# mmeidlinger/lut_ldpc

Measured on AMD Instinct MI355X. Metric: decoded codewords/sec, DVB-S2 N=64800 4-bit LUT 50-iter, higher is better.
Workload: dtype u8

## Files before the change

lut_ldpc_amd/csrc/hip/kernels_common.hpp:

```cpp
#pragma once
#ifndef __HIPCC_RTC__
#include <hip/hip_runtime.h>
#include <stdint.h>
#else
typedef unsigned char uint8_t;
typedef unsigned short uint16_t;
typedef unsigned int uint32_t;
typedef unsigned long long uint64_t;
typedef short int16_t;
typedef int int32_t;
typedef long long int64_t;
#endif

namespace lutldpc {

constexpr int kRowBytes = 256;
constexpr int kTileFrames = kRowBytes;
constexpr int kWave = 64;
constexpr int kMaxSeg = 32;

constexpr uint32_t ST_ACTIVE = 0, ST_DONE_PSC = 1, ST_DONE_PISC = 2, ST_PAD = 3;
constexpr uint32_t ST_DONE_SAVED = 4;

struct PassSeg {
    int32_t block_begin;
    int32_t n_nodes;
    int32_t node_off;
    int32_t deg;
    int32_t op_off;
    int32_t n_ops;
    int32_t tab_off;
    int32_t tab_bytes;
    int32_t n_in, n_out, n_slots;
    int32_t fast;
};

struct PassParams {
    int32_t n_seg;
    int32_t blocks_per_group;
    int32_t nodes_per_block;
    int32_t G;
    int32_t E;
    int32_t N;
    int32_t nz;
    int32_t check;
    int32_t write_hard;
    int32_t slots_lds;
    int32_t vfail_stride_w;
    PassSeg seg[kMaxSeg];
};

template <int PACK>
__device__ __forceinline__ uint32_t unpack_half(uint32_t x, int h) {
    if constexpr (PACK == 1) return x;
    else return h ? ((x >> 4) & 0x0F0F0F0Fu) : (x & 0x0F0F0F0Fu);
}
template <int PACK>
__device__ __forceinline__ uint32_t pack_halves(const uint32_t (&r)[PACK]) {
    if constexpr (PACK == 1) return r[0];
    else return r[0] | (r[1] << 4);
}
template <int PACK>
__device__ __forceinline__ uint32_t pack_masks(const uint32_t (&m)[PACK]) {
    if constexpr (PACK == 1) return m[0];
    else return (m[0] & 0x0F0F0F0Fu) | (m[1] & 0xF0F0F0F0u);
}
template <int PACK>
__device__ __forceinline__ int frame_word(int g, int lane, int h) { return (g * kWave + lane) * PACK + h; }

__device__ __forceinline__ uint32_t swar_lt(uint32_t x, uint32_t t) {
    uint32_t d = (x | 0x80808080u) - t * 0x01010101u;
    return (~d >> 7) & 0x01010101u;
}
__device__ __forceinline__ uint32_t swar_zero_mask(uint32_t x) {
    uint32_t nz = ((x & 0x7F7F7F7Fu) + 0x7F7F7F7Fu) | x;
    uint32_t z = (~nz >> 7) & 0x01010101u;
    return z * 0xFFu;
}
__device__ __forceinline__ uint32_t bfi(uint32_t m, uint32_t a, uint32_t b) { return __builtin_amdgcn_bitop3_b32(m, a, b, (0xCC & 0xF0) | (0xAA & 0x0F)); }

using rsrc_t = __amdgpu_buffer_rsrc_t;
__device__ __forceinline__ rsrc_t make_rsrc(const void *p, uint32_t bytes) {
    return __builtin_amdgcn_make_buffer_rsrc(const_cast<void *>(p), 0, (int)bytes, 0x00020000);
}
#ifndef LUTLDPC_LD_AUX
#define LUTLDPC_LD_AUX 2
#endif
#ifndef LUTLDPC_ST_AUX
#define LUTLDPC_ST_AUX 2
#endif
__device__ __forceinline__ uint32_t ld_row(rsrc_t r, uint32_t row_off, uint32_t lane4) {
    return (uint32_t)__builtin_amdgcn_raw_buffer_load_b32(r, (int)lane4, (int)row_off, LUTLDPC_LD_AUX);
}
__device__ __forceinline__ void st_row(rsrc_t r, uint32_t row_off, uint32_t lane4, uint32_t v) {
    __builtin_amdgcn_raw_buffer_store_b32(v, r, (int)lane4, (int)row_off, LUTLDPC_ST_AUX);
}

__device__ __forceinline__ void pipeline_entry_fence() {
    asm volatile("" ::: "memory");
    __builtin_amdgcn_sched_barrier(0);
    __builtin_amdgcn_s_waitcnt(0x0F70);
    __builtin_amdgcn_sched_barrier(0);
    asm volatile("" ::: "memory");
}

__device__ __forceinline__ bool wave_all_zero(uint32_t x) { return __ballot(x != 0) == 0ull; }

template <int PACK>
__device__ __forceinline__ bool load_active(const uint32_t *__restrict__ state_w, int g, int lane, uint32_t (&amask)[PACK]) {
    uint32_t any = 0;
#pragma unroll
    for (int h = 0; h < PACK; h++) { amask[h] = swar_zero_mask(state_w[frame_word<PACK>(g, lane, h)]); any |= amask[h]; }
    return wave_all_zero(any);
}

template <int PACK>
__device__ __forceinline__ void store_blend(uint32_t *p, uint32_t val, uint32_t old, uint32_t smask) {
    *p = bfi(smask, val, old);
}
template <int PACK>
__device__ __forceinline__ void store_row_masked(uint32_t *p, uint32_t val, uint32_t smask) {
    if (smask == 0xFFFFFFFFu) *p = val;
    else if (smask) *p = bfi(smask, val, *p);
}

constexpr int kVfailSlots = 32;
template <int PACK>
__device__ __forceinline__ void flag_frames(uint32_t *__restrict__ vfail_w, int stride_w, int g, int lane, const uint32_t (&fail)[PACK], const uint32_t (&amask)[PACK]) {
    uint32_t *slot = vfail_w + (size_t)(blockIdx.x & (kVfailSlots - 1)) * (size_t)stride_w;
#pragma unroll
    for (int h = 0; h < PACK; h++) {
        const uint32_t f = fail[h] & amask[h] & 0x01010101u;
        if (f) atomicOr(&slot[frame_word<PACK>(g, lane, h)], f);
    }
}

constexpr int kFastMaxTables = 32;
constexpr int kFastTableStride = 256;

struct FastParams {
    int32_t n_nodes, node_off, nodes_per_wave, waves_per_group;
    int32_t idx_off;
    int32_t G, E, N;
    int32_t g0;
    int32_t nz;
    int32_t shift_msg;
    int32_t check, write_hard;
    int32_t deg;
    int32_t n_tables;
    int32_t tab_off[kFastMaxTables];
    int32_t tab_len[kFastMaxTables];
    int32_t tab_shift[kFastMaxTables];
    int32_t nib;
    int32_t vfail_stride_w;
    int32_t vfail_off_w;
};
struct ChainParams {
    int32_t on;
    int32_t idx_off;
    int32_t tab_off, tab_len, tab_shift;
    int32_t check, hard, vfail_off_w, sbit_out;
};

__device__ __forceinline__ uint32_t lshl_or(uint32_t x, int s, uint32_t y) {
    uint32_t r;
    asm("v_lshl_or_b32 %0, %1, %2, %3" : "=v"(r) : "v"(x), "s"(s), "v"(y));
    return r;
}

__device__ __forceinline__ uint32_t xad(uint32_t a, uint32_t b, uint32_t c) {
    uint32_t r;
    asm("v_xad_u32 %0, %1, %2, %3" : "=v"(r) : "v"(a), "s"(b), "v"(c));
    return r;
}
__device__ __forceinline__ uint32_t xor3(uint32_t a, uint32_t b, uint32_t c) { return __builtin_amdgcn_bitop3_b32(a, b, c, 0xF0 ^ 0xCC ^ 0xAA); }
__device__ __forceinline__ uint32_t xor_or(uint32_t a, uint32_t b, uint32_t c) { return __builtin_amdgcn_bitop3_b32(a, b, c, (0xF0 ^ 0xCC) | 0xAA); }

#ifndef __HIPCC_RTC__
constexpr size_t kMaxKernelArgBytes = 128;
template <typename... KArgs, typename... Args>
inline void launch_k(void (*kernel)(KArgs...), dim3 grid, dim3 block, size_t shmem, hipStream_t stream, Args &&...args) {
    static_assert((((sizeof(KArgs) + 7) / 8 * 8) + ... + 0) <= kMaxKernelArgBytes, "kernel argument segment above 128 bytes: pass the structure through device memory");
    hipLaunchKernelGGL(kernel, grid, block, shmem, stream, static_cast<KArgs>(args)...);
}
#endif

__device__ __forceinline__ int find_seg(const PassParams &P, int b) {
    int s = 0;
#pragma unroll 1
    for (int i = 1; i < P.n_seg; i++) if (b >= P.seg[i].block_begin) s = i;
    return s;
}

}
```

lut_ldpc_amd/csrc/hip/kernels_fast.hpp:

```cpp
#pragma once
#include "kernels_common.hpp"
#include "lut_program.hpp"

#include <utility>

namespace lutldpc {

constexpr int kCnAllButOneMaxDeg = 16;
template <int DEG, int UNR, int PACK, bool CHAIN, typename PT, bool FIRST = false, int ABO = kCnAllButOneMaxDeg>
__device__ __forceinline__ void cn_minsum_body(
    const PT &P, int block, uint8_t *msgs, const uint32_t *__restrict__ state_w, uint32_t *__restrict__ vfail_w,
    const int32_t *__restrict__ fast_idx, const ChainParams CH = ChainParams{}, uint8_t *lds_tab = nullptr,
    const uint8_t *cha = nullptr, const uint8_t *__restrict__ tables = nullptr, uint8_t *hard = nullptr, const uint8_t *msg0 = nullptr)
{
    static_assert(!CHAIN || (UNR == 1 && DEG >= 2), "chain fusion: one check per step");
    if constexpr (CHAIN) {
        const int i = threadIdx.x;
        if (CH.on && i < CH.tab_len / 4) reinterpret_cast<uint32_t *>(lds_tab)[i] = reinterpret_cast<const uint32_t *>(tables + CH.tab_off)[i];
        __syncthreads();
    }
    const int lane = threadIdx.x & 63;
    const int wave = __builtin_amdgcn_readfirstlane(block * 4 + (threadIdx.x >> 6));
    const int gl = wave / P.waves_per_group;
    if (gl >= P.G) return;
    const int chunk = wave - gl * P.waves_per_group;
    const int g = gl + P.g0;
    uint32_t amask[PACK];
    if (load_active<PACK>(state_w, g, lane, amask)) return;
    const uint32_t smask = pack_masks<PACK>(amask);
    const bool all_active = __ballot(smask != 0xFFFFFFFFu) == 0ull;
    const rsrc_t base = make_rsrc(msgs + (size_t)g * (size_t)P.E * kRowBytes, (uint32_t)P.E * kRowBytes);
    const uint32_t lane4 = (uint32_t)lane * 4u;
    const int32_t *edges = fast_idx + P.idx_off;
    const int32_t *nodes = edges;
    rsrc_t nbase = base;
    if constexpr (FIRST) {
        nodes = fast_idx + P.nidx_off;
        nbase = make_rsrc(msg0 + (size_t)g * (size_t)P.N * kRowBytes, (uint32_t)P.N * kRowBytes);
    }
    const int first = chunk * P.nodes_per_wave;
    int last = first + P.nodes_per_wave;
    if (last > P.n_nodes) last = P.n_nodes;
    constexpr uint32_t ONE = PACK == 2 ? 0x11111111u : 0x01010101u;
    const int sbit = __builtin_ctz((unsigned)P.nz);
    const uint32_t SB = (uint32_t)P.nz * ONE, LOW = SB - ONE;
    const uint32_t odd = (DEG & 1) ? SB : 0u;
    uint32_t failw = 0;

    const int32_t *links = CHAIN ? fast_idx + CH.idx_off : nullptr;
    const rsrc_t cbase = CHAIN ? make_rsrc(cha + (size_t)g * (size_t)P.N * kRowBytes, (uint32_t)P.N * kRowBytes) : base;
    int lb = 0, lf = 0, lbn = 0, lfn = 0;
    uint32_t xc = 0, xcn = 0;
    uint32_t pend = 0, pend_old = 0, chainfail = 0;
    int pend_e = 0;
    auto fetch = [&](int i, uint32_t (&xx)[UNR][DEG], int (&ee)[UNR][DEG]) {
#pragma unroll
        for (int u = 0; u < UNR; u++) {
            const int ii = (i + u < last) ? i + u : last - 1;
#pragma unroll
            for (int k = 0; k < DEG; k++) ee[u][k] = edges[(size_t)ii * DEG + k];
            if constexpr (CHAIN) { lbn = links[2 * (size_t)ii]; lfn = links[2 * (size_t)ii + 1]; }
        }
#pragma unroll
        for (int u = 0; u < UNR; u++) {
            const uint32_t off = lane4 | ((i + u < last) ? 0u : 0x80000000u);
#pragma unroll
            for (int k = 0; k < DEG; k++) {
                if constexpr (FIRST) {
                    const int ii = (i + u < last) ? i + u : last - 1;
                    xx[u][k] = ld_row(nbase, (uint32_t)nodes[(size_t)ii * DEG + k] * kRowBytes, off);
                } else xx[u][k] = ld_row(base, (uint32_t)ee[u][k] * kRowBytes, off);
            }
            if constexpr (CHAIN) xcn = ld_row(cbase, (uint32_t)(lbn > 0 ? lbn - 1 : 0) * kRowBytes, (i + u < last && lbn > 0 && CH.on) ? lane4 : (lane4 | 0x80000000u));
        }
    };
    auto to_mc = [&](uint32_t xh) -> uint32_t {
        const uint32_t pos = xh & SB;
        return (xh ^ (pos - (pos >> sbit))) & LOW;
    };
    auto from_mc = [&](uint32_t mc, uint32_t po) -> uint32_t {
        return xor_or(mc, po - (po >> sbit), po);
    };
    auto eval = [&](int i, const uint32_t (&x)[UNR][DEG], const int (&e)[UNR][DEG]) {
#pragma unroll
        for (int u = 0; u < UNR; u++) {
            if (i + u >= last) break;
            uint32_t r[DEG];
            uint32_t tn;
            if constexpr (DEG <= ABO) {
            auto mx = [&](uint32_t a, uint32_t b) -> uint32_t {
                const uint32_t gt = xad(b, LOW, a) & SB;
                return bfi(gt - (gt >> sbit), a, b);
            };
            uint32_t mcs[DEG], spp = 0;
#pragma unroll
            for (int k = 0; k < DEG; k++) {
                const uint32_t xh = x[u][k];
                mcs[k] = to_mc(xh);
                if (k & 1) spp = xor3(spp, x[u][k - 1], xh);
                else if (k == DEG - 1) spp ^= xh;
            }
            tn = (spp ^ odd) & SB;
            uint32_t oc[DEG];
            if constexpr (DEG == 1) oc[0] = 0u;
            else if constexpr (DEG == 2) { oc[0] = mcs[1]; oc[1] = mcs[0]; }
            else {
                uint32_t suf[DEG];
                suf[DEG - 1] = mcs[DEG - 1];
#pragma unroll
                for (int k = DEG - 2; k >= 1; k--) suf[k] = mx(mcs[k], suf[k + 1]);
                uint32_t pre = mcs[0];
                oc[0] = suf[1];
#pragma unroll
                for (int k = 1; k <= DEG - 2; k++) { oc[k] = mx(pre, suf[k + 1]); pre = mx(pre, mcs[k]); }
                oc[DEG - 1] = pre;
            }
#pragma unroll
            for (int k = 0; k < DEG; k++) r[k] = from_mc(oc[k], (tn ^ x[u][k]) & SB);
            } else {
            uint32_t min1 = LOW, min2 = LOW, spp = 0;
            uint32_t mg[DEG];
#pragma unroll
            for (int k = 0; k < DEG; k++) {
                const uint32_t xh = x[u][k];
                const uint32_t mag = to_mc(xh) ^ LOW;
                spp ^= xh;
                mg[k] = mag;
                if (k == 0) {
                    min1 = mag;
                } else {
                    const uint32_t g1 = ((mag | SB) - min1) & SB;
                    const uint32_t k1 = g1 - (g1 >> sbit);
                    const uint32_t lo = bfi(k1, min1, mag);
                    const uint32_t hi = mag ^ min1 ^ lo;
                    if (k == 1) {
                        min2 = hi;
                    } else {
                        const uint32_t g2 = ((min2 | SB) - hi) & SB;
                        const uint32_t k2 = g2 - (g2 >> sbit);
                        min2 = bfi(k2, hi, min2);
                    }
                    min1 = lo;
                }
            }
            tn = (spp ^ odd) & SB;
            const uint32_t m1c = min1 ^ LOW, m2c = min2 ^ LOW;
#pragma unroll
            for (int k = 0; k < DEG; k++) {
                const uint32_t eq = ~(((mg[k] ^ min1) | SB) - ONE) & SB;
                const uint32_t ke = eq - (eq >> sbit);
                r[k] = from_mc(bfi(ke, m2c, m1c), (tn ^ x[u][k]) & SB);
            }
            }
            if (P.check) failw |= tn >> sbit;
            if constexpr (CHAIN) {
                [[maybe_unused]] constexpr int F = 4 * PACK, BITS = 8 / PACK;
                if (lb && CH.hard) {
                    const uint32_t neg = (~x[u][0] >> sbit) & ONE;
                    store_row_masked<PACK>(reinterpret_cast<uint32_t *>(hard + ((size_t)g * (size_t)P.N + (size_t)(lb - 1)) * kRowBytes + lane4), neg, smask);
                }
                if (lb && CH.on) {
                    uint32_t o_prev = 0, o_this = 0, dif = 0;
                    if constexpr (PACK == 2) {
                        constexpr uint32_t NIB = 0x0F0F0F0Fu;
                        const uint32_t c_lo = xc & NIB, c_hi = (xc >> 4) & NIB;
                        const uint32_t ia_lo = lshl_or(c_lo, CH.tab_shift, pend & NIB), ia_hi = lshl_or(c_hi, CH.tab_shift, (pend >> 4) & NIB);
                        const uint32_t ib_lo = lshl_or(c_lo, CH.tab_shift, r[0] & NIB), ib_hi = lshl_or(c_hi, CH.tab_shift, (r[0] >> 4) & NIB);
#pragma unroll 1
                        for (int s = 0; s < 32; s += 8) {
                            const uint32_t vp0 = lds_tab[__builtin_amdgcn_ubfe(ib_lo, (uint32_t)s, 8u)], vt0 = lds_tab[__builtin_amdgcn_ubfe(ia_lo, (uint32_t)s, 8u)];
                            const uint32_t vp1 = lds_tab[__builtin_amdgcn_ubfe(ib_hi, (uint32_t)s, 8u)], vt1 = lds_tab[__builtin_amdgcn_ubfe(ia_hi, (uint32_t)s, 8u)];
                            o_prev = lshl_or(vp0, s, o_prev);
                            o_this = lshl_or(vt0, s, o_this);
                            o_prev = lshl_or(vp1, s + 4, o_prev);
                            o_this = lshl_or(vt1, s + 4, o_this);
                        }
                    } else {
#pragma unroll 1
                    for (int s = 0; s < F * BITS; s += 2 * BITS) {
#pragma unroll
                        for (int t = 0; t < 2; t++) {
                            const int sb = s + t * BITS;
                            const uint32_t a = __builtin_amdgcn_ubfe(pend, (uint32_t)sb, (uint32_t)BITS), b = __builtin_amdgcn_ubfe(r[0], (uint32_t)sb, (uint32_t)BITS);
                            const uint32_t c = __builtin_amdgcn_ubfe(xc, (uint32_t)sb, (uint32_t)BITS);
                            const uint32_t vp = lds_tab[lshl_or(c, CH.tab_shift, b)], vt = lds_tab[lshl_or(c, CH.tab_shift, a)];
                            o_prev = lshl_or(vp, sb, o_prev);
                            o_this = lshl_or(vt, sb, o_this);
                        }
                    }
                    }
                    if (CH.check) dif = ((o_prev ^ o_this) >> CH.sbit_out) & ONE;
                    chainfail |= dif;
                    st_row(base, (uint32_t)__builtin_amdgcn_readfirstlane(pend_e) * kRowBytes, lane4, bfi(smask, o_prev, pend_old));
                    r[0] = o_this;
                }
                if (lf && CH.on) { pend = r[1]; pend_e = e[u][1]; pend_old = x[u][1]; }
#pragma unroll
                for (int k = 0; k < DEG; k++)
                    if (!(k == 1 && lf && CH.on)) st_row(base, (uint32_t)e[u][k] * kRowBytes, lane4, bfi(smask, r[k], x[u][k]));
            } else if (all_active) {
#pragma unroll
                for (int k = 0; k < DEG; k++) st_row(base, (uint32_t)e[u][k] * kRowBytes, lane4, r[k]);
            } else {
#pragma unroll
                for (int k = 0; k < DEG; k++) st_row(base, (uint32_t)e[u][k] * kRowBytes, lane4, bfi(smask, r[k], x[u][k]));
            }
        }
    };
    if constexpr (DEG <= 16) {
        uint32_t x[UNR][DEG], xn[UNR][DEG];
        int e[UNR][DEG], en[UNR][DEG];
        fetch(first, x, e);
        if constexpr (CHAIN) { lb = lbn; lf = lfn; xc = xcn; }
        fetch(first + UNR, xn, en);
        eval(first, x, e);
        pipeline_entry_fence();
        for (int i = first + UNR; i < last; i += UNR) {
#pragma unroll
            for (int u = 0; u < UNR; u++)
#pragma unroll
                for (int k = 0; k < DEG; k++) { x[u][k] = xn[u][k]; e[u][k] = en[u][k]; }
            if constexpr (CHAIN) { lb = lbn; lf = lfn; xc = xcn; }
            fetch(i + UNR, xn, en);
            eval(i, x, e);
        }
    } else {
        for (int i = first; i < last; i += UNR) {
            uint32_t x[UNR][DEG];
            int e[UNR][DEG];
            fetch(i, x, e);
            if constexpr (CHAIN) { lb = lbn; lf = lfn; xc = xcn; }
            eval(i, x, e);
        }
    }
    if (P.check) {
        uint32_t fail[PACK];
#pragma unroll
        for (int h = 0; h < PACK; h++) fail[h] = unpack_half<PACK>(failw, h);
        flag_frames<PACK>(vfail_w + P.vfail_off_w, P.vfail_stride_w, g, lane, fail, amask);
    }
    if constexpr (CHAIN) {
        if (CH.check && CH.on) {
            uint32_t fail[PACK];
#pragma unroll
            for (int h = 0; h < PACK; h++) fail[h] = unpack_half<PACK>(chainfail, h);
            flag_frames<PACK>(vfail_w + CH.vfail_off_w, P.vfail_stride_w, g, lane, fail, amask);
        }
    }
}

template <int DEG, int UNR, int PACK>
__global__ __launch_bounds__(256) void cn_minsum_fast_kernel(
    const FastParams *__restrict__ Pp, uint8_t *__restrict__ msgs, const uint32_t *__restrict__ state_w, uint32_t *__restrict__ vfail_w,
    const int32_t *__restrict__ fast_idx)
{
    const FastParams &P = *Pp;
    cn_minsum_body<DEG, UNR, PACK, false>(P, (int)blockIdx.x, msgs, state_w, vfail_w, fast_idx);
}

template <int N>
struct BalShape {
    static constexpr int NI = N > 1 ? N - 1 : 0;
    int left[NI > 0 ? NI : 1] = {};
    int right[NI > 0 ? NI : 1] = {};
    int size[2 * N] = {};
    int first[2 * N] = {};
    int off[NI > 0 ? NI : 1] = {};
    int top = 0;
    int total = 0;
};

template <int N>
constexpr BalShape<N> make_bal_shape() {
    BalShape<N> S{};
    int fifo[2 * N + 2] = {};
    int head = 0, tail = 0, next = N;
    for (int l = 0; l < N; l++) { fifo[tail++] = l; S.size[l] = 1; }
    while (tail - head > 1) {
        const int a = fifo[head++], b = fifo[head++];
        S.left[next - N] = a; S.right[next - N] = b;
        S.size[next] = S.size[a] + S.size[b];
        fifo[tail++] = next++;
    }
    S.top = fifo[head];
    int stack[2 * N + 2] = {};
    int sp = 0, pos = 0;
    stack[sp++] = S.top;
    while (sp > 0) {
        const int nd = stack[--sp];
        S.first[nd] = pos;
        if (nd < N) { pos += 1; continue; }
        stack[sp++] = S.right[nd - N];
        stack[sp++] = S.left[nd - N];
    }
    int total = 0;
    for (int j = 0; j < BalShape<N>::NI; j++) { S.off[j] = total; total += S.size[N + j] + 1; }
    S.total = total;
    return S;
}


__device__ __forceinline__ uint32_t lut1(const uint8_t *lds_tab, int t, uint32_t a, uint32_t b, int sh) {
    return lds_tab[t * kFastTableStride + lshl_or(b, sh, a)];
}

template <int N, int C, int KC>
__device__ __forceinline__ uint32_t bal_child(const uint32_t *in, const uint32_t *v) {
    constexpr BalShape<N> S = make_bal_shape<N>();
    if constexpr (C < N) { constexpr int idx = S.first[C] + (KC ? 0 : 1); return in[idx]; }
    else { constexpr int idx = S.off[C - N] + KC; return v[idx]; }
}

template <int N, int J, int K>
__device__ __forceinline__ void bal_node_variant(const uint32_t *in, uint32_t *v, const uint8_t *tab, int sh) {
    constexpr BalShape<N> S = make_bal_shape<N>();
    constexpr int L = S.left[J], R = S.right[J], sl = S.size[L];
    constexpr int kl = K < sl ? K : sl, kr = K > sl ? K - sl : 0;
    constexpr int dst = S.off[J] + K;
    v[dst] = lut1(tab, J, bal_child<N, L, kl>(in, v), bal_child<N, R, kr>(in, v), sh);
}

template <int N, int J, int... Ks>
__device__ __forceinline__ void bal_node_all(const uint32_t *in, uint32_t *v, const uint8_t *tab, int sh, std::integer_sequence<int, Ks...>) {
    (bal_node_variant<N, J, Ks>(in, v, tab, sh), ...);
}
template <int N, bool ALL, int... Js>
__device__ __forceinline__ void bal_all_nodes(const uint32_t *in, uint32_t *v, const uint8_t *tab, int sh, std::integer_sequence<int, Js...>) {
    if constexpr (ALL) (bal_node_all<N, Js>(in, v, tab, sh, std::make_integer_sequence<int, make_bal_shape<N>().size[N + Js] + 1>{}), ...);
    else (bal_node_variant<N, Js, make_bal_shape<N>().size[N + Js]>(in, v, tab, sh), ...);
}

template <int DV, int KIND, bool CHECK, int PACK, typename PT>
__device__ __forceinline__ void vn_balanced_body(
    const PT &P, int block, uint8_t *lds_tab, uint8_t *msgs, const uint8_t *cha, uint8_t *__restrict__ hard,
    const uint32_t *__restrict__ state_w, uint32_t *__restrict__ vfail_w, const uint8_t *__restrict__ tables,
    const int32_t *__restrict__ fast_idx)
{
    constexpr int N = (KIND == TT_DEC) ? DV : DV - 1;
    constexpr int NI = N > 1 ? N - 1 : 0;
    constexpr int NB = N > 1 ? N : 2;
    {
        uint32_t tmp[NI + 1];
        const int i = threadIdx.x;
#pragma unroll
        for (int t = 0; t <= NI; t++) tmp[t] = (i < P.tab_len[t] / 4) ? reinterpret_cast<const uint32_t *>(tables + P.tab_off[t])[i] : 0u;
#pragma unroll
        for (int t = 0; t <= NI; t++) if (i < P.tab_len[t] / 4) reinterpret_cast<uint32_t *>(lds_tab + t * kFastTableStride)[i] = tmp[t];
    }
    __syncthreads();

    const int lane = threadIdx.x & 63;
    const int wave = __builtin_amdgcn_readfirstlane(block * 4 + (threadIdx.x >> 6));
    const int gl = wave / P.waves_per_group;
    if (gl >= P.G) return;
    const int chunk = wave - gl * P.waves_per_group;
    const int g = gl + P.g0;
    uint32_t amask[PACK];
    if (load_active<PACK>(state_w, g, lane, amask)) return;
    const uint32_t smask = pack_masks<PACK>(amask);
    const int32_t *vtab = fast_idx + P.idx_off;
    const rsrc_t mbase = make_rsrc(msgs + (size_t)g * (size_t)P.E * kRowBytes, (uint32_t)P.E * kRowBytes);
    const rsrc_t cbase = make_rsrc(cha + (size_t)g * (size_t)P.N * kRowBytes, (uint32_t)P.N * kRowBytes);
    uint8_t *hbase = hard + (size_t)g * (size_t)P.N * kRowBytes;
    const uint32_t lane4 = (uint32_t)lane * 4u;
    const int first = chunk * P.nodes_per_wave;
    int last = first + P.nodes_per_wave;
    if (last > P.n_nodes) last = P.n_nodes;
    const int sh = P.shift_msg, shr = P.tab_shift[NI];
    const int sbit = (KIND == TT_VAR && CHECK) ? __builtin_ctz((unsigned)P.nz | 0x100u) : 0;
    uint32_t failw = 0;

    auto fetch = [&](int i, int &vv, int &ee, uint32_t (&r)[DV + 1]) {
        const int ic = i < last ? i : last - 1;
        vv = vtab[2 * (size_t)ic]; ee = vtab[2 * (size_t)ic + 1];
        const uint32_t off = lane4 | (i < last ? 0u : 0x80000000u);
#pragma unroll
        for (int k = 0; k < DV; k++) r[k] = ld_row(mbase, (uint32_t)(ee + k) * kRowBytes, off);
        r[DV] = ld_row(cbase, (uint32_t)vv * kRowBytes, off);
    };
    auto eval = [&](const uint32_t (&raw)[DV + 1], int v, int e0) {
        constexpr int F = 4 * PACK, BITS = 8 / PACK;
        constexpr int U = DV <= 8 ? 2 : 1;
        constexpr BalShape<NB> SH = make_bal_shape<NB>();
        constexpr int top_off = SH.off[SH.top - NB];
        uint32_t out[DV], hardw = 0;
#pragma unroll
        for (int o = 0; o < DV; o++) out[o] = 0;
#pragma unroll 1
        for (int sp = 0; sp < F * BITS; sp += U * BITS) {
#pragma unroll
            for (int u = 0; u < U; u++) {
                const int s = sp + u * BITS;
                uint32_t in[DV + 1];
#pragma unroll
                for (int k = 0; k <= DV; k++) in[k] = __builtin_amdgcn_ubfe(raw[k], (uint32_t)s, (uint32_t)BITS);
                const uint32_t ch = in[DV];
                uint32_t val[(N > 1 ? SH.total : 1)];
                if constexpr (N > 1) bal_all_nodes<N, KIND == TT_VAR>(in, val, lds_tab, sh, std::make_integer_sequence<int, NI>{});
                if constexpr (KIND == TT_DEC) {
                    uint32_t top;
                    if constexpr (N > 1) top = val[top_off + N];
                    else top = in[0];
                    hardw = lshl_or(lut1(lds_tab, NI, top, ch, shr) < 1u ? 1u : 0u, s, hardw);
                } else {
#pragma unroll
                    for (int o = 0; o < DV; o++) {
                        uint32_t r;
                        if constexpr (N == 0) {
                            r = lut1(lds_tab, 0, ch, 0u, 0);
                        } else {
                            uint32_t top;
                            if constexpr (N > 1) top = val[top_off + o];
                            else top = in[o == 0 ? 1 : 0];
                            r = lut1(lds_tab, NI, top, ch, shr);
                        }
                        out[o] = lshl_or(r, s, out[o]);
                    }
                }
            }
        }
        if constexpr (KIND == TT_VAR && CHECK) {
            constexpr uint32_t ONE = PACK == 2 ? 0x11111111u : 0x01010101u;
            uint32_t diff = 0;
#pragma unroll
            for (int o = 1; o < DV; o++) diff |= out[o] ^ out[0];
            failw |= (diff >> sbit) & ONE;
            if (P.write_hard) hardw = (~out[0] >> sbit) & ONE;
        }
        if constexpr (KIND == TT_DEC) {
            store_row_masked<PACK>(reinterpret_cast<uint32_t *>(hbase + (size_t)v * kRowBytes + lane4), hardw, smask);
        } else {
#pragma unroll
            for (int o = 0; o < DV; o++) st_row(mbase, (uint32_t)(e0 + o) * kRowBytes, lane4, bfi(smask, out[o], raw[o]));
            if (CHECK && P.write_hard)
                store_row_masked<PACK>(reinterpret_cast<uint32_t *>(hbase + (size_t)v * kRowBytes + lane4), hardw, smask);
        }
    };
    int v, e0, vn, en;
    uint32_t raw[DV + 1], nxt[DV + 1];
    fetch(first, v, e0, raw);
    fetch(first + 1, vn, en, nxt);
    eval(raw, v, e0);
    pipeline_entry_fence();
    for (int i = first + 1; i < last; i++) {
#pragma unroll
        for (int k = 0; k <= DV; k++) raw[k] = nxt[k];
        v = vn; e0 = en;
        fetch(i + 1, vn, en, nxt);
        eval(raw, v, e0);
    }
    if (KIND == TT_VAR && CHECK) {
        uint32_t fail[PACK];
#pragma unroll
        for (int h = 0; h < PACK; h++) fail[h] = unpack_half<PACK>(failw, h);
        flag_frames<PACK>(vfail_w + P.vfail_off_w, P.vfail_stride_w, g, lane, fail, amask);
    }
}

template <int DV, int KIND, bool CHECK, int PACK>
__global__ __launch_bounds__(256) void vn_balanced_fast_kernel(
    const FastParams *__restrict__ Pp, uint8_t *msgs, const uint8_t *cha, uint8_t *__restrict__ hard,
    const uint32_t *__restrict__ state_w, uint32_t *__restrict__ vfail_w, const uint8_t *__restrict__ tables,
    const int32_t *__restrict__ fast_idx)
{
    constexpr int NT = (KIND == TT_DEC ? DV : DV - 1) > 1 ? (KIND == TT_DEC ? DV : DV - 1) : 1;
    __shared__ __attribute__((aligned(16))) uint8_t lds_tab[NT * kFastTableStride];
    const FastParams &P = *Pp;
    vn_balanced_body<DV, KIND, CHECK, PACK>(P, (int)blockIdx.x, lds_tab, msgs, cha, hard, state_w, vfail_w, tables, fast_idx);
}

#ifndef LUTLDPC_B0_WAVES_MIN
#define LUTLDPC_B0_WAVES_MIN 7
#endif
#ifndef LUTLDPC_B0_WAVES_MAX
#define LUTLDPC_B0_WAVES_MAX 8
#endif
constexpr int kFusedMaxRoles = 10;
constexpr int kFusedMaxTables = 20;
constexpr int kFusedBuckets = 4;
constexpr int kFusedVnDeg[kFusedBuckets] = {8, 12, 20, 8};
constexpr int kFusedCnDeg[kFusedBuckets] = {8, 16, 32, 10};
constexpr int kFusedAboDeg[kFusedBuckets] = {8, 10, 16, 8};
constexpr int kFusedBucketOrder[kFusedBuckets] = {0, 3, 1, 2};
inline int fused_bucket(int max_vn_deg, int max_cn_deg) {
    for (int b : kFusedBucketOrder) if (max_vn_deg <= kFusedVnDeg[b] && max_cn_deg <= kFusedCnDeg[b]) return b;
    return -1;
}
inline int fused_bucket_rank(int bucket) { for (int i = 0; i < kFusedBuckets; i++) if (kFusedBucketOrder[i] == bucket) return i; return -1; }
inline constexpr int fused_max_cn_deg() { int m = 0; for (int b = 0; b < kFusedBuckets; b++) m = kFusedCnDeg[b] > m ? kFusedCnDeg[b] : m; return m; }

struct RoleParams {
    int32_t kind;
    int32_t deg;
    int32_t g0, G;
    int32_t n_nodes, nodes_per_wave, waves_per_group, idx_off;
    int32_t E, N, nz, shift_msg, check, write_hard;
    int32_t vfail_stride_w, vfail_off_w;
    int32_t first, nidx_off;
    ChainParams chain;
    int32_t tab_off[kFusedMaxTables], tab_len[kFusedMaxTables], tab_shift[kFusedMaxTables];
};
struct FusedParams {
    int32_t n_roles;
    int32_t prio;
    RoleParams role[kFusedMaxRoles];
};

template <int PACK, bool CHAIN, bool FIRST, int ABO, int... Ds>
__device__ __forceinline__ void fused_cn_switch(const RoleParams &P, int block, std::integer_sequence<int, Ds...>, uint8_t *msgs, const uint32_t *state_w,
                                                uint32_t *vfail_w, const int32_t *fast_idx, uint8_t *lds_tab, const uint8_t *cha, const uint8_t *tables, uint8_t *hard,
                                                const uint8_t *msg0) {
    ((P.deg == Ds + 2 ? (cn_minsum_body<Ds + 2, 1, PACK, CHAIN, RoleParams, FIRST, ABO>(P, block, msgs, state_w, vfail_w, fast_idx, P.chain, lds_tab, cha, tables, hard, msg0), 0) : 0), ...);
}
template <int PACK, bool CHECK, int... Ds>
__device__ __forceinline__ void fused_vn_switch(const RoleParams &P, int block, std::integer_sequence<int, Ds...>, uint8_t *lds_tab, uint8_t *msgs,
                                                const uint8_t *cha, uint8_t *hard, const uint32_t *state_w, uint32_t *vfail_w, const uint8_t *tables,
                                                const int32_t *fast_idx) {
    ((P.deg == Ds + 1 ? (vn_balanced_body<Ds + 1, TT_VAR, CHECK, PACK>(P, block, lds_tab, msgs, cha, hard, state_w, vfail_w, tables, fast_idx), 0) : 0), ...);
}

template <int PACK, bool CHECK, int BUCKET>
__global__ __launch_bounds__(256) __attribute__((amdgpu_waves_per_eu((BUCKET == 0 || BUCKET == 3) ? LUTLDPC_B0_WAVES_MIN : BUCKET == 1 ? 4 : 3, (BUCKET == 0 || BUCKET == 3) ? LUTLDPC_B0_WAVES_MAX : 8))) void pass_fused_kernel(
    const RoleParams *__restrict__ roles, const int2 *__restrict__ items, int prio, uint8_t *msgs, const uint8_t *cha, uint8_t *__restrict__ hard,
    const uint32_t *__restrict__ state_w, uint32_t *__restrict__ vfail_w, const uint8_t *__restrict__ tables, const int32_t *__restrict__ fast_idx,
    const uint8_t *__restrict__ msg0)
{
    constexpr int MAXVN = kFusedVnDeg[BUCKET], MAXCN = kFusedCnDeg[BUCKET];
    __shared__ __attribute__((aligned(16))) uint8_t lds_tab[MAXVN * kFastTableStride];
    const int2 it = items[blockIdx.x];
    const int r = __builtin_amdgcn_readfirstlane(it.x), rb = __builtin_amdgcn_readfirstlane(it.y);
    const RoleParams &P = roles[r];
    if (prio && P.kind) {
        if (P.deg >= 4) __builtin_amdgcn_s_setprio(3); else __builtin_amdgcn_s_setprio(1);
    }
    if (P.kind == 0) {
        constexpr auto degs = std::make_integer_sequence<int, MAXCN - 1>{};
        if (!P.first) {
            if (P.chain.on || P.chain.hard) fused_cn_switch<PACK, true, false, kFusedAboDeg[BUCKET]>(P, rb, degs, msgs, state_w, vfail_w, fast_idx, lds_tab, cha, tables, hard, msg0);
            else fused_cn_switch<PACK, false, false, kFusedAboDeg[BUCKET]>(P, rb, degs, msgs, state_w, vfail_w, fast_idx, lds_tab, cha, tables, hard, msg0);
        } else {
            if (P.chain.on) fused_cn_switch<PACK, true, true, kFusedAboDeg[BUCKET]>(P, rb, degs, msgs, state_w, vfail_w, fast_idx, lds_tab, cha, tables, hard, msg0);
            else fused_cn_switch<PACK, false, true, kFusedAboDeg[BUCKET]>(P, rb, degs, msgs, state_w, vfail_w, fast_idx, lds_tab, cha, tables, hard, msg0);
        }
    }
    else fused_vn_switch<PACK, CHECK>(P, rb, std::make_integer_sequence<int, MAXVN>{}, lds_tab, msgs, cha, hard, state_w, vfail_w, tables, fast_idx);
}

inline bool match_balanced(const Tree &t, int kind, int d, std::vector<const TreeNode *> &canon) {
    canon.clear();
    const int n = (kind == TT_DEC) ? d : d - 1;
    const TreeNode *root = t.root.get();
    if (!root || root->type != NT_ROOT) return false;
    if (n == 0) {
        if (root->child.size() != 1 || root->child[0]->type != NT_CHA) return false;
        canon.push_back(root);
        return true;
    }
    if (root->child.size() != 2 || root->child[1]->type != NT_CHA || !root->child[1]->child.empty()) return false;
    std::vector<int> left, right, fifo;
    for (int l = 0; l < n; l++) fifo.push_back(l);
    size_t head = 0;
    int next = n;
    while (fifo.size() - head > 1) {
        left.push_back(fifo[head]); right.push_back(fifo[head + 1]);
        head += 2;
        fifo.push_back(next++);
    }
    const int top = fifo[head];
    std::vector<const TreeNode *> node_of((size_t)(2 * n), nullptr);
    struct Item { int id; const TreeNode *tn; };
    std::vector<Item> stack{{top, root->child[0].get()}};
    while (!stack.empty()) {
        Item it = stack.back(); stack.pop_back();
        if (it.id < n) {
            if (it.tn->type != NT_MSG || !it.tn->child.empty()) return false;
            continue;
        }
        if (it.tn->type != NT_IM || it.tn->child.size() != 2) return false;
        node_of[(size_t)it.id] = it.tn;
        stack.push_back({right[(size_t)(it.id - n)], it.tn->child[1].get()});
        stack.push_back({left[(size_t)(it.id - n)], it.tn->child[0].get()});
    }
    for (int j = n; j < 2 * n - 1; j++) { if (!node_of[(size_t)j]) return false; canon.push_back(node_of[(size_t)j]); }
    canon.push_back(root);
    return true;
}

inline bool is_pow2(int x) { return x > 0 && (x & (x - 1)) == 0; }

struct FastClassPlan {
    bool ok = false;
    FastParams P{};
};

inline FastClassPlan plan_fast_vn(const Tree &t, int kind, int d, const std::map<const TreeNode *, std::pair<uint32_t, uint32_t>> &tab_of, int node_off, int n_nodes) {
    FastClassPlan fp;
    std::vector<const TreeNode *> canon;
    if (d < 1 || d > 20 || !match_balanced(t, kind, d, canon) || (int)canon.size() > kFastMaxTables) return fp;
    int shift_msg = -1;
    for (size_t j = 0; j < canon.size(); j++) {
        const TreeNode *nd = canon[j];
        auto it = tab_of.find(nd);
        if (it == tab_of.end() || it->second.second > 256u) return fp;
        for (auto &c : nd->child) if (!is_pow2(c->K) || c->K > 128) return fp;
        if (!is_pow2(nd->K) || nd->K > 128) return fp;
        const int sh0 = __builtin_ctz((unsigned)nd->child[0]->K);
        if (j + 1 < canon.size()) {
            if (nd->child[0]->K != nd->child[1]->K) return fp;
            if (shift_msg < 0) shift_msg = sh0; else if (shift_msg != sh0) return fp;
        }
        fp.P.tab_off[j] = (int32_t)it->second.first;
        fp.P.tab_len[j] = (int32_t)it->second.second;
        fp.P.tab_shift[j] = sh0;
    }
    fp.P.shift_msg = shift_msg < 0 ? 0 : shift_msg;
    fp.P.n_tables = (int)canon.size();
    fp.P.nib = 0;
    fp.P.deg = d; fp.P.node_off = node_off; fp.P.n_nodes = n_nodes;
    fp.ok = true;
    return fp;
}

constexpr int kFastMaxDeg = 20;
constexpr int kFastMaxCnDeg = 32;

template <int KIND, bool CHECK, int PACK, int DV>
void launch_vn_fast_one(hipStream_t s, const FastParams &P, const FastParams *dP, uint8_t *msgs, const uint8_t *cha, uint8_t *hard, const uint32_t *state_w,
                        uint32_t *vfail_w, const uint8_t *tables, const int32_t *fast_idx) {
    const int waves = P.waves_per_group * P.G;
    launch_k(vn_balanced_fast_kernel<DV, KIND, CHECK, PACK>, dim3((unsigned)((waves + 3) / 4)), dim3(256), 0, s, dP, msgs, cha, hard, state_w, vfail_w,
             tables, fast_idx);
}

template <int KIND, bool CHECK, int PACK, int... DVs>
bool dispatch_vn_fast(int deg, std::integer_sequence<int, DVs...>, hipStream_t s, const FastParams &P, const FastParams *dP, uint8_t *msgs, const uint8_t *cha,
                      uint8_t *hard, const uint32_t *state_w, uint32_t *vfail_w, const uint8_t *tables, const int32_t *fast_idx) {
    bool done = false;
    ((deg == DVs + 1 ? (launch_vn_fast_one<KIND, CHECK, PACK, DVs + 1>(s, P, dP, msgs, cha, hard, state_w, vfail_w, tables, fast_idx), done = true) : false), ...);
    return done;
}

inline void fill_vn_fast(FastParams &P, int G, int nz, int check, int write_hard, int nodes_per_wave, int E, int N, int vfail_stride_w) {
    P.vfail_stride_w = vfail_stride_w;
    P.G = G; P.E = E; P.N = N; P.nz = nz; P.check = check; P.write_hard = write_hard;
    P.nodes_per_wave = nodes_per_wave;
    P.waves_per_group = (P.n_nodes + nodes_per_wave - 1) / nodes_per_wave;
}
template <int KIND, int PACK>
bool launch_vn_fast(hipStream_t s, const FastParams &P, const FastParams *dP, uint8_t *msgs, const uint8_t *cha,
                    uint8_t *hard, const uint32_t *state_w, uint32_t *vfail_w, const uint8_t *tables, const int32_t *fast_idx) {
    constexpr auto seq = std::make_integer_sequence<int, kFastMaxDeg>{};
    if (KIND == TT_VAR && P.check) return dispatch_vn_fast<KIND, true, PACK>(P.deg, seq, s, P, dP, msgs, cha, hard, state_w, vfail_w, tables, fast_idx);
    return dispatch_vn_fast<KIND, false, PACK>(P.deg, seq, s, P, dP, msgs, cha, hard, state_w, vfail_w, tables, fast_idx);
}

template <int PACK, int DEG>
void launch_cn_fast_one(hipStream_t s, const FastParams &P, const FastParams *dP, uint8_t *msgs, const uint32_t *state_w, uint32_t *vfail_w, const int32_t *fast_idx) {
    constexpr int UNR = DEG <= 4 ? 4 : DEG <= 10 ? 2 : 1;
    const int waves = P.waves_per_group * P.G;
    launch_k(cn_minsum_fast_kernel<DEG, UNR, PACK>, dim3((unsigned)((waves + 3) / 4)), dim3(256), 0, s, dP, msgs, state_w, vfail_w, fast_idx);
}
template <int PACK, int... Ds>
bool dispatch_cn_fast(int deg, std::integer_sequence<int, Ds...>, hipStream_t s, const FastParams &P, const FastParams *dP, uint8_t *msgs, const uint32_t *state_w,
                      uint32_t *vfail_w, const int32_t *fast_idx) {
    bool done = false;
    ((deg == Ds + 1 ? (launch_cn_fast_one<PACK, Ds + 1>(s, P, dP, msgs, state_w, vfail_w, fast_idx), done = true) : false), ...);
    return done;
}

inline bool fill_cn_fast(FastParams &P, int deg, int n_nodes, int idx_off, int G, int E, int nz, int check, int nodes_per_wave, int vfail_stride_w) {
    if (!is_pow2(nz) || nz > 64 || deg < 2 || deg > kFastMaxCnDeg) return false;
    P = FastParams{};
    P.n_nodes = n_nodes; P.idx_off = idx_off; P.G = G; P.E = E; P.nz = nz; P.check = check; P.deg = deg; P.vfail_stride_w = vfail_stride_w;
    P.nodes_per_wave = nodes_per_wave;
    P.waves_per_group = (n_nodes + nodes_per_wave - 1) / nodes_per_wave;
    return true;
}
template <int PACK>
bool launch_cn_fast(hipStream_t s, const FastParams &P, const FastParams *dP, uint8_t *msgs, const uint32_t *state_w, uint32_t *vfail_w, const int32_t *fast_idx) {
    return dispatch_cn_fast<PACK>(P.deg, std::make_integer_sequence<int, kFastMaxCnDeg>{}, s, P, dP, msgs, state_w, vfail_w, fast_idx);
}

template <int KIND, int PACK>
hipError_t preload_vn_fast() {
    hipFuncAttributes a;
    return hipFuncGetAttributes(&a, reinterpret_cast<const void *>(&vn_balanced_fast_kernel<2, KIND, false, PACK>));
}
template <int PACK>
hipError_t preload_cn_fast() {
    hipFuncAttributes a;
    return hipFuncGetAttributes(&a, reinterpret_cast<const void *>(&cn_minsum_fast_kernel<2, 4, PACK>));
}

template <int PACK, int BUCKET>
void launch_fused(hipStream_t s, const RoleParams *d_roles, const int32_t *items, int n_blocks, int prio, bool vn_check, uint8_t *msgs, const uint8_t *cha, uint8_t *hard,
                  const uint32_t *state_w, uint32_t *vfail_w, const uint8_t *tables, const int32_t *fast_idx, const uint8_t *msg0) {
    if (vn_check)
        launch_k(pass_fused_kernel<PACK, true, BUCKET>, dim3((unsigned)n_blocks), dim3(256), 0, s, d_roles, reinterpret_cast<const int2 *>(items), prio, msgs, cha, hard,
                 state_w, vfail_w, tables, fast_idx, msg0);
    else
        launch_k(pass_fused_kernel<PACK, false, BUCKET>, dim3((unsigned)n_blocks), dim3(256), 0, s, d_roles, reinterpret_cast<const int2 *>(items), prio, msgs, cha, hard,
                 state_w, vfail_w, tables, fast_idx, msg0);
}
template <int PACK, int BUCKET>
hipError_t preload_fused() {
    hipFuncAttributes a;
    return hipFuncGetAttributes(&a, reinterpret_cast<const void *>(&pass_fused_kernel<PACK, false, BUCKET>));
}

#define LUTLDPC_FUSED_SIG (hipStream_t, const RoleParams *, const int32_t *, int, int, bool, uint8_t *, const uint8_t *, uint8_t *, const uint32_t *, uint32_t *, const uint8_t *, const int32_t *, const uint8_t *)
#define LUTLDPC_FAST_LAUNCHERS(X)                                                                                                           \
    X template bool launch_vn_fast<TT_VAR, 1>(hipStream_t, const FastParams &, const FastParams *, uint8_t *, const uint8_t *, uint8_t *, const uint32_t *, uint32_t *, const uint8_t *, const int32_t *); \
    X template bool launch_vn_fast<TT_VAR, 2>(hipStream_t, const FastParams &, const FastParams *, uint8_t *, const uint8_t *, uint8_t *, const uint32_t *, uint32_t *, const uint8_t *, const int32_t *); \
    X template bool launch_vn_fast<TT_DEC, 1>(hipStream_t, const FastParams &, const FastParams *, uint8_t *, const uint8_t *, uint8_t *, const uint32_t *, uint32_t *, const uint8_t *, const int32_t *); \
    X template bool launch_vn_fast<TT_DEC, 2>(hipStream_t, const FastParams &, const FastParams *, uint8_t *, const uint8_t *, uint8_t *, const uint32_t *, uint32_t *, const uint8_t *, const int32_t *); \
    X template bool launch_cn_fast<1>(hipStream_t, const FastParams &, const FastParams *, uint8_t *, const uint32_t *, uint32_t *, const int32_t *);    \
    X template bool launch_cn_fast<2>(hipStream_t, const FastParams &, const FastParams *, uint8_t *, const uint32_t *, uint32_t *, const int32_t *);    \
    X template void launch_fused<1, 0> LUTLDPC_FUSED_SIG; X template void launch_fused<2, 0> LUTLDPC_FUSED_SIG; \
    X template void launch_fused<1, 1> LUTLDPC_FUSED_SIG; X template void launch_fused<2, 1> LUTLDPC_FUSED_SIG; \
    X template void launch_fused<1, 2> LUTLDPC_FUSED_SIG; X template void launch_fused<2, 2> LUTLDPC_FUSED_SIG; \
    X template void launch_fused<1, 3> LUTLDPC_FUSED_SIG; X template void launch_fused<2, 3> LUTLDPC_FUSED_SIG; \
    X template hipError_t preload_fused<2, 0>(); X template hipError_t preload_fused<2, 1>(); X template hipError_t preload_fused<2, 2>(); X template hipError_t preload_fused<2, 3>(); \
    X template hipError_t preload_vn_fast<TT_VAR, 1>(); X template hipError_t preload_vn_fast<TT_VAR, 2>(); X template hipError_t preload_vn_fast<TT_DEC, 2>(); \
    X template hipError_t preload_cn_fast<2>();

}
```

Before: 261,900.

## Overlap LUT table staging and state load with first message-row fetch

```diff
diff --git a/lut_ldpc_amd/csrc/hip/kernels_common.hpp b/lut_ldpc_amd/csrc/hip/kernels_common.hpp
--- a/lut_ldpc_amd/csrc/hip/kernels_common.hpp
+++ b/lut_ldpc_amd/csrc/hip/kernels_common.hpp
@@ -111,6 +111,19 @@
     uint32_t any = 0;
 #pragma unroll
     for (int h = 0; h < PACK; h++) { amask[h] = swar_zero_mask(state_w[frame_word<PACK>(g, lane, h)]); any |= amask[h]; }
+    return wave_all_zero(any);
+}
+
+template <int PACK>
+__device__ __forceinline__ void load_state_words(const uint32_t *__restrict__ state_w, int g, int lane, uint32_t (&sw)[PACK]) {
+#pragma unroll
+    for (int h = 0; h < PACK; h++) sw[h] = state_w[frame_word<PACK>(g, lane, h)];
+}
+template <int PACK>
+__device__ __forceinline__ bool active_from_words(const uint32_t (&sw)[PACK], uint32_t (&amask)[PACK]) {
+    uint32_t any = 0;
+#pragma unroll
+    for (int h = 0; h < PACK; h++) { amask[h] = swar_zero_mask(sw[h]); any |= amask[h]; }
     return wave_all_zero(any);
 }
 
diff --git a/lut_ldpc_amd/csrc/hip/kernels_fast.hpp b/lut_ldpc_amd/csrc/hip/kernels_fast.hpp
--- a/lut_ldpc_amd/csrc/hip/kernels_fast.hpp
+++ b/lut_ldpc_amd/csrc/hip/kernels_fast.hpp
@@ -14,21 +14,14 @@
     const uint8_t *cha = nullptr, const uint8_t *__restrict__ tables = nullptr, uint8_t *hard = nullptr, const uint8_t *msg0 = nullptr)
 {
     static_assert(!CHAIN || (UNR == 1 && DEG >= 2), "chain fusion: one check per step");
-    if constexpr (CHAIN) {
-        const int i = threadIdx.x;
-        if (CH.on && i < CH.tab_len / 4) reinterpret_cast<uint32_t *>(lds_tab)[i] = reinterpret_cast<const uint32_t *>(tables + CH.tab_off)[i];
-        __syncthreads();
-    }
     const int lane = threadIdx.x & 63;
     const int wave = __builtin_amdgcn_readfirstlane(block * 4 + (threadIdx.x >> 6));
-    const int gl = wave / P.waves_per_group;
-    if (gl >= P.G) return;
-    const int chunk = wave - gl * P.waves_per_group;
+    const int gl_raw = wave / P.waves_per_group;
+    const bool idle = gl_raw >= P.G;
+    if constexpr (!CHAIN) { if (idle) return; }
+    const int gl = idle ? 0 : gl_raw;
+    const int chunk = idle ? 0 : wave - gl * P.waves_per_group;
     const int g = gl + P.g0;
-    uint32_t amask[PACK];
-    if (load_active<PACK>(state_w, g, lane, amask)) return;
-    const uint32_t smask = pack_masks<PACK>(amask);
-    const bool all_active = __ballot(smask != 0xFFFFFFFFu) == 0ull;
     const rsrc_t base = make_rsrc(msgs + (size_t)g * (size_t)P.E * kRowBytes, (uint32_t)P.E * kRowBytes);
     const uint32_t lane4 = (uint32_t)lane * 4u;
     const int32_t *edges = fast_idx + P.idx_off;
@@ -53,7 +46,7 @@
     uint32_t xc = 0, xcn = 0;
     uint32_t pend = 0, pend_old = 0, chainfail = 0;
     int pend_e = 0;
-    auto fetch = [&](int i, uint32_t (&xx)[UNR][DEG], int (&ee)[UNR][DEG]) {
+    auto fetch = [&](int i, uint32_t (&xx)[UNR][DEG], int (&ee)[UNR][DEG], bool dead = false) {
 #pragma unroll
         for (int u = 0; u < UNR; u++) {
             const int ii = (i + u < last) ? i + u : last - 1;
@@ -63,7 +56,7 @@
         }
 #pragma unroll
         for (int u = 0; u < UNR; u++) {
-            const uint32_t off = lane4 | ((i + u < last) ? 0u : 0x80000000u);
+            const uint32_t off = lane4 | ((i + u < last && !dead) ? 0u : 0x80000000u);
 #pragma unroll
             for (int k = 0; k < DEG; k++) {
                 if constexpr (FIRST) {
@@ -71,9 +64,26 @@
                     xx[u][k] = ld_row(nbase, (uint32_t)nodes[(size_t)ii * DEG + k] * kRowBytes, off);
                 } else xx[u][k] = ld_row(base, (uint32_t)ee[u][k] * kRowBytes, off);
             }
-            if constexpr (CHAIN) xcn = ld_row(cbase, (uint32_t)(lbn > 0 ? lbn - 1 : 0) * kRowBytes, (i + u < last && lbn > 0 && CH.on) ? lane4 : (lane4 | 0x80000000u));
+            if constexpr (CHAIN) xcn = ld_row(cbase, (uint32_t)(lbn > 0 ? lbn - 1 : 0) * kRowBytes, (i + u < last && lbn > 0 && CH.on && !dead) ? lane4 : (lane4 | 0x80000000u));
         }
     };
+    uint32_t x[UNR][DEG];
+    int e[UNR][DEG];
+    uint32_t sw[PACK], tabw = 0;
+    load_state_words<PACK>(state_w, g, lane, sw);
+    [[maybe_unused]] const bool stage = CHAIN && CH.on && (int)threadIdx.x < CH.tab_len / 4;
+    if constexpr (CHAIN) { if (stage) tabw = reinterpret_cast<const uint32_t *>(tables + CH.tab_off)[threadIdx.x]; }
+    constexpr bool EARLY = DEG <= 16;
+    if constexpr (EARLY) fetch(first, x, e, idle);
+    if constexpr (CHAIN) {
+        if (stage) reinterpret_cast<uint32_t *>(lds_tab)[threadIdx.x] = tabw;
+        __syncthreads();
+        if (idle) return;
+    }
+    uint32_t amask[PACK];
+    if (active_from_words<PACK>(sw, amask)) return;
+    const uint32_t smask = pack_masks<PACK>(amask);
+    const bool all_active = __ballot(smask != 0xFFFFFFFFu) == 0ull;
     auto to_mc = [&](uint32_t xh) -> uint32_t {
         const uint32_t pos = xh & SB;
         return (xh ^ (pos - (pos >> sbit))) & LOW;
@@ -208,9 +218,8 @@
         }
     };
     if constexpr (DEG <= 16) {
-        uint32_t x[UNR][DEG], xn[UNR][DEG];
-        int e[UNR][DEG], en[UNR][DEG];
-        fetch(first, x, e);
+        uint32_t xn[UNR][DEG];
+        int en[UNR][DEG];
         if constexpr (CHAIN) { lb = lbn; lf = lfn; xc = xcn; }
         fetch(first + UNR, xn, en);
         eval(first, x, e);
@@ -226,8 +235,6 @@
         }
     } else {
         for (int i = first; i < last; i += UNR) {
-            uint32_t x[UNR][DEG];
-            int e[UNR][DEG];
             fetch(i, x, e);
             if constexpr (CHAIN) { lb = lbn; lf = lfn; xc = xcn; }
             eval(i, x, e);
@@ -339,25 +346,13 @@
     constexpr int N = (KIND == TT_DEC) ? DV : DV - 1;
     constexpr int NI = N > 1 ? N - 1 : 0;
     constexpr int NB = N > 1 ? N : 2;
-    {
-        uint32_t tmp[NI + 1];
-        const int i = threadIdx.x;
-#pragma unroll
-        for (int t = 0; t <= NI; t++) tmp[t] = (i < P.tab_len[t] / 4) ? reinterpret_cast<const uint32_t *>(tables + P.tab_off[t])[i] : 0u;
-#pragma unroll
-        for (int t = 0; t <= NI; t++) if (i < P.tab_len[t] / 4) reinterpret_cast<uint32_t *>(lds_tab + t * kFastTableStride)[i] = tmp[t];
-    }
-    __syncthreads();
-
     const int lane = threadIdx.x & 63;
     const int wave = __builtin_amdgcn_readfirstlane(block * 4 + (threadIdx.x >> 6));
-    const int gl = wave / P.waves_per_group;
-    if (gl >= P.G) return;
-    const int chunk = wave - gl * P.waves_per_group;
+    const int gl_raw = wave / P.waves_per_group;
+    const bool idle = gl_raw >= P.G;
+    const int gl = idle ? 0 : gl_raw;
+    const int chunk = idle ? 0 : wave - gl * P.waves_per_group;
     const int g = gl + P.g0;
-    uint32_t amask[PACK];
-    if (load_active<PACK>(state_w, g, lane, amask)) return;
-    const uint32_t smask = pack_masks<PACK>(amask);
     const int32_t *vtab = fast_idx + P.idx_off;
     const rsrc_t mbase = make_rsrc(msgs + (size_t)g * (size_t)P.E * kRowBytes, (uint32_t)P.E * kRowBytes);
     const rsrc_t cbase = make_rsrc(cha + (size_t)g * (size_t)P.N * kRowBytes, (uint32_t)P.N * kRowBytes);
@@ -370,14 +365,30 @@
     const int sbit = (KIND == TT_VAR && CHECK) ? __builtin_ctz((unsigned)P.nz | 0x100u) : 0;
     uint32_t failw = 0;
 
-    auto fetch = [&](int i, int &vv, int &ee, uint32_t (&r)[DV + 1]) {
+    auto fetch = [&](int i, int &vv, int &ee, uint32_t (&r)[DV + 1], bool dead = false) {
         const int ic = i < last ? i : last - 1;
         vv = vtab[2 * (size_t)ic]; ee = vtab[2 * (size_t)ic + 1];
-        const uint32_t off = lane4 | (i < last ? 0u : 0x80000000u);
+        const uint32_t off = lane4 | ((i < last && !dead) ? 0u : 0x80000000u);
 #pragma unroll
         for (int k = 0; k < DV; k++) r[k] = ld_row(mbase, (uint32_t)(ee + k) * kRowBytes, off);
         r[DV] = ld_row(cbase, (uint32_t)vv * kRowBytes, off);
     };
+    int v, e0, vn, en;
+    uint32_t raw[DV + 1], nxt[DV + 1];
+    uint32_t amask[PACK];
+    {
+        uint32_t sw[PACK], tmp[NI + 1];
+        const int i = threadIdx.x;
+        load_state_words<PACK>(state_w, g, lane, sw);
+#pragma unroll
+        for (int t = 0; t <= NI; t++) tmp[t] = (i < P.tab_len[t] / 4) ? reinterpret_cast<const uint32_t *>(tables + P.tab_off[t])[i] : 0u;
+        fetch(first, v, e0, raw, idle);
+#pragma unroll
+        for (int t = 0; t <= NI; t++) if (i < P.tab_len[t] / 4) reinterpret_cast<uint32_t *>(lds_tab + t * kFastTableStride)[i] = tmp[t];
+        __syncthreads();
+        if (idle || active_from_words<PACK>(sw, amask)) return;
+    }
+    const uint32_t smask = pack_masks<PACK>(amask);
     auto eval = [&](const uint32_t (&raw)[DV + 1], int v, int e0) {
         constexpr int F = 4 * PACK, BITS = 8 / PACK;
         constexpr int U = DV <= 8 ? 2 : 1;
@@ -436,9 +447,6 @@
                 store_row_masked<PACK>(reinterpret_cast<uint32_t *>(hbase + (size_t)v * kRowBytes + lane4), hardw, smask);
         }
     };
-    int v, e0, vn, en;
-    uint32_t raw[DV + 1], nxt[DV + 1];
-    fetch(first, v, e0, raw);
     fetch(first + 1, vn, en, nxt);
     eval(raw, v, e0);
     pipeline_entry_fence();
```

Result: slower. 259,000 (-1.1%).
